# routineLife1/DRBA

Hardware: AMD Instinct MI355X
Metric: interpolated frames/sec @1080p RIFE x2 (higher is better)
Workload: dtype f32 (2xfp16-term MFMA operands = 22 significand bits, fp32 accumulate)

## Files before the change

drba_amd/csrc/conv_split.hip:

```cpp
#include "common.hpp"
#include "conv_split.hpp"

#include <string.h>

#include <map>
#include <mutex>
#include <type_traits>
#include <utility>

using namespace drba;

namespace drba_conv_split {

typedef float f32x4 __attribute__((ext_vector_type(4)));
typedef __bf16 bf16x8 __attribute__((ext_vector_type(8)));
typedef _Float16 f16x8 __attribute__((ext_vector_type(8)));
typedef unsigned u32x4 __attribute__((ext_vector_type(4)));

constexpr int CK = 32;

template <int MODE_, int RW_, int MW_, int NT_, int PL_ = 3, int CS_ = 1, int BP_ = 0>
struct SplitCfg {
  static constexpr int MODE = MODE_, RW = RW_, MW = MW_, NT = NT_, PL = PL_, CS = CS_;
  static constexpr bool BP = BP_ != 0;
  static_assert(!BP || MODE == 1, "row phases exist in the transposed form only");
  static constexpr int NTT = NT * CS;
  static constexpr int NTAP = MODE != 1 ? 9 : 4, NPX = MODE != 1 ? 1 : (BP ? 4 : 2);
  static constexpr int TH = (4 / CS) * RW, TW = 16 * MW, NTC = 16 * NTT;
  static constexpr int TR = MODE == 2 ? 2 * TH + 1 : TH + 2, TC = MODE == 2 ? 2 * TW + 1 : TW + 2, NPIX = TR * TC;
  static constexpr int NPIXP = ((NPIX + 15) / 16) * 16 + 4;
  static constexpr int LDS_BYTES = PL * 4 * NPIXP * 16;
  static constexpr int ITEMS = NPIX * 4;
  static constexpr int LIT = (ITEMS + 255) / 256;
  static constexpr int FRAG_U4 = NTAP * NTT * PL * 64;
#ifndef DRBA_SPLIT_BDEPTH_BIG
#define DRBA_SPLIT_BDEPTH_BIG 2
#endif
#ifndef DRBA_SPLIT_BDEPTH2_BIG
#define DRBA_SPLIT_BDEPTH2_BIG 2
#endif
#ifndef DRBA_SPLIT_BDEPTH2_SMALL
#define DRBA_SPLIT_BDEPTH2_SMALL 4
#endif
  static constexpr int BDEPTH = PL == 3 ? ((RW * MW >= 4) ? DRBA_SPLIT_BDEPTH_BIG : 4)
                                        : ((RW * MW >= 4) ? DRBA_SPLIT_BDEPTH2_BIG : DRBA_SPLIT_BDEPTH2_SMALL);
#ifndef DRBA_SPLIT_MINB3
#define DRBA_SPLIT_MINB3 1
#endif
  static constexpr int MINB = (DRBA_SPLIT_MINB3 && MODE == 0 && RW * MW * NT <= 4 && PL == 3 && CS == 1) ? 3 : 2;
};

__device__ __forceinline__ void split2(float a, float b, unsigned &h, unsigned &m, unsigned &l) {
  typedef __bf16 bf16x2 __attribute__((ext_vector_type(2)));
  typedef float f32x2 __attribute__((ext_vector_type(2)));
  auto pk = [](float x, float y) -> unsigned {
    const bf16x2 p = __builtin_convertvector(f32x2{x, y}, bf16x2);
    return __builtin_bit_cast(unsigned, p);
  };
  h = pk(a, b);
  const float ra = a - __uint_as_float(h << 16), rb = b - __uint_as_float(h & 0xffff0000u);
  m = pk(ra, rb);
  l = pk(ra - __uint_as_float(m << 16), rb - __uint_as_float(m & 0xffff0000u));
}

constexpr int kActShift = drba::kSplitActShift;
__device__ __forceinline__ void split2_f16(float a, float b, unsigned &h, unsigned &l) {
  typedef _Float16 f16x2 __attribute__((ext_vector_type(2)));
  typedef float f32x2 __attribute__((ext_vector_type(2)));
  const f32x2 v = (f32x2){a, b} * (1.f / (float)(1 << kActShift));
  const f16x2 hh = __builtin_convertvector(v, f16x2);
  const f32x2 r = (v - __builtin_convertvector(hh, f32x2)) * 2048.f;
  const f16x2 ll = __builtin_convertvector(r, f16x2);
  h = __builtin_bit_cast(unsigned, hh);
  l = __builtin_bit_cast(unsigned, ll);
}

struct TileCtx {
  int x0, y0, cz, n, py;
};

#ifdef DRBA_PHASE_CLOCKS
__device__ long long g_phase[1024 * 4 * 4];
#define DRBA_CLK(var) const long long var = (long long)__builtin_readcyclecounter()
#define DRBA_CLK_ADD(slot, a, b) clk_acc[slot] += (b) - (a)
#define DRBA_CLK_INIT long long clk_acc[4] = {0, 0, 0, 0}
#define DRBA_CLK_FLUSH                                                                     \
  if (lane == 0 && blockIdx.x < 1024) {                                                    \
    for (int k_ = 0; k_ < 4; ++k_) g_phase[(blockIdx.x * 4 + wave) * 4 + k_] += clk_acc[k_]; \
  }
#else
#define DRBA_CLK(var)
#define DRBA_CLK_ADD(slot, a, b)
#define DRBA_CLK_INIT
#define DRBA_CLK_FLUSH
#endif

__device__ __forceinline__ void lds_barrier() { asm volatile("s_waitcnt lgkmcnt(0)\n\ts_barrier" ::: "memory"); }

template <class Cfg, bool PRE, bool RL = false, bool PSH = false>
__global__ void __launch_bounds__(256, Cfg::MINB)
conv_split_mfma(const float *__restrict__ in, const u32x4 *__restrict__ wfrag, const float *__restrict__ bias,
                const float *__restrict__ beta, const float *__restrict__ res, const float *__restrict__ res2,
                float *__restrict__ out, int Cin, int H, int W, int Cout, int act, float post_slope, float pre_slope,
                int n_ctiles, int nbx, int nby, int total, int pixel_shuffle, int Hi, int Wi, unsigned char *status) {
#if defined(__HIP_DEVICE_COMPILE__)
  constexpr int MODE = Cfg::MODE, NTAP = Cfg::NTAP, NPX = Cfg::NPX;
  constexpr int RW = Cfg::RW, MW = Cfg::MW, NT = Cfg::NT, TH = Cfg::TH, TW = Cfg::TW, TC = Cfg::TC;
  constexpr int NPIX = Cfg::NPIX, NPIXP = Cfg::NPIXP, LIT = Cfg::LIT, PL = Cfg::PL;
  static_assert(PL == 3 || !RL, "the residual is rebuilt exactly only from the three bf16 planes");
  extern __shared__ __attribute__((aligned(16))) u32x4 tile[];

  const int tid = threadIdx.x, lane = tid & 63;
  const int wave = __builtin_amdgcn_readfirstlane(tid >> 6);
  const int m = lane & 15, kq = lane >> 4;
  const size_t HW = (size_t)H * W, HWi = (size_t)Hi * Wi;
  const int nchunks = (Cin + CK - 1) / CK;
  constexpr int CS = Cfg::CS, NTT = Cfg::NTT;
  const int row0 = (CS == 1 ? wave : wave % (4 / CS)) * RW;
  const int nt0 = CS == 1 ? 0 : (wave / (4 / CS)) * NT;

  auto decode = [&](int work) -> TileCtx {
    int t = xcd_band(work, total);
    TileCtx c;
    c.py = 0;
    if (MODE == 1 && !Cfg::BP) {
      c.py = t & 1;
      t >>= 1;
    }
    c.cz = t % n_ctiles;
    t /= n_ctiles;
    const int bx = t % nbx;
    t /= nbx;
    c.x0 = bx * TW, c.y0 = (t % nby) * TH, c.n = t / nby;
    return c;
  };

  const unsigned img_bytes = (unsigned)((size_t)Cin * HWi * 4);
  const __amdgpu_buffer_rsrc_t wrsrc =
      __builtin_amdgcn_make_buffer_rsrc((void *)wfrag, 0, n_ctiles * (MODE != 1 ? 1 : 4) * nchunks * Cfg::FRAG_U4 * 16, 0x00020000);
  float pre[LIT][8];
  auto fetch = [&](const TileCtx &c, int q) {
    const __amdgpu_buffer_rsrc_t irsrc =
        __builtin_amdgcn_make_buffer_rsrc((void *)(in + (size_t)c.n * Cin * HWi), 0, img_bytes, 0x00020000);
    const int plane = (int)HWi * 4;
#pragma unroll
    for (int it = 0; it < LIT; ++it) {
      const int item = tid + 256 * it;
      const int g = item / NPIX, p = item - g * NPIX;
      const int r = p / TC, cc = p - r * TC;
      const int y = (MODE == 2 ? 2 * c.y0 : c.y0) + r - 1, x = (MODE == 2 ? 2 * c.x0 : c.x0) + cc - 1;
      const bool ok = item < Cfg::ITEMS && y >= 0 && y < Hi && x >= 0 && x < Wi;
      const unsigned voff = ok ? (unsigned)(g * 8 * plane + (y * Wi + x) * 4) : 0xffffffffu;
#pragma unroll
      for (int i = 0; i < 8; ++i)
        pre[it][i] = __builtin_bit_cast(float, __builtin_amdgcn_raw_buffer_load_b32(irsrc, voff, (q * CK + i) * plane, 0));
    }
  };
  auto stage = [&]() {
#pragma unroll
    for (int it = 0; it < LIT; ++it) {
      const int item = tid + 256 * it;
      if (item >= Cfg::ITEMS) continue;
      const int g = item / NPIX, slot = g * NPIXP + (item - g * NPIX);
      u32x4 h, mm, l;
#pragma unroll
      for (int i = 0; i < 4; ++i) {
        float a = pre[it][2 * i], b = pre[it][2 * i + 1];
        if (PRE) {
          a = a > 0.f ? a : a * pre_slope;
          b = b > 0.f ? b : b * pre_slope;
        }
        unsigned hh, hm = 0, hl;
        if constexpr (PL == 3) split2(a, b, hh, hm, hl);
        else split2_f16(a, b, hh, hl);
        h[i] = hh, mm[i] = hm, l[i] = hl;
      }
      tile[slot] = h;
      if constexpr (PL == 3) tile[4 * NPIXP + slot] = mm;
      tile[4 * (PL - 1) * NPIXP + slot] = l;
    }
  };

  const bool vec = !PSH && (W & 3) == 0 && (MW & 1) == 0;

  int work = blockIdx.x;
  if (work >= total) return;
  DRBA_CLK_INIT;
  float nf = 0.f;
#ifdef DRBA_SPLIT_STAGGER
  {
    const int b = blockIdx.x;
    const bool late = DRBA_SPLIT_STAGGER == 1 ? (b & 1) : DRBA_SPLIT_STAGGER == 2 ? (b >= (int)gridDim.x / 2) : DRBA_SPLIT_STAGGER == 4 ? ((b >> 8) & 1) : ((b >> 3) & 1);
    if (late) {
      for (int i = 0; i < DRBA_SPLIT_STAGGER_N; ++i) __builtin_amdgcn_s_sleep(127);
    }
  }
#endif
  TileCtx ctx = decode(work);
  auto first_chunk = [&](const TileCtx &c) -> int { return RL ? (c.cz + 1 == nchunks ? 0 : c.cz + 1) : 0; };
  fetch(ctx, first_chunk(ctx));
  while (true) {
    f32x4 acc[NPX][RW][MW][NT];
    f32x4 acl[PL == 2 ? NPX : 1][RW][MW][NT];
#pragma unroll
    for (int p = 0; p < NPX; ++p)
#pragma unroll
      for (int a = 0; a < RW; ++a)
#pragma unroll
        for (int b = 0; b < MW; ++b)
#pragma unroll
          for (int c = 0; c < NT; ++c) {
            acc[p][a][b][c] = (f32x4){0.f, 0.f, 0.f, 0.f};
            if constexpr (PL == 2) acl[p][a][b][c] = (f32x4){0.f, 0.f, 0.f, 0.f};
          }
    const int next = work + (int)gridDim.x;
    TileCtx nctx = ctx;
    if (next < total) nctx = decode(next);
    const bool regroup = MODE != 1 && vec;
    float bs[NT], bt[NT], bs2[NT], bt2[NT];
#pragma unroll
    for (int nt = 0; nt < NT; ++nt) {
      const int co = ctx.cz * Cfg::NTC + (nt0 + nt) * 16 + (regroup ? (lane >> 3) : m), co2 = co + 8;
      bs[nt] = (bias && co < Cout) ? bias[co] : 0.f;
      bt[nt] = (beta && co < Cout) ? beta[co] : 0.f;
      bs2[nt] = (regroup && bias && co2 < Cout) ? bias[co2] : 0.f;
      bt2[nt] = (regroup && beta && co2 < Cout) ? beta[co2] : 0.f;
    }

    for (int qi = 0; qi < nchunks; ++qi) {
      int q = qi;
      if (RL) {
        q = qi + first_chunk(ctx);
        if (q >= nchunks) q -= nchunks;
      }
      constexpr int NTS = NPX * NTAP, STEPS = NTS * NT, D = Cfg::BDEPTH;
      const int wq = ((MODE != 1 ? ctx.cz : ctx.cz * 4 + 2 * ctx.py) * nchunks + q) * (Cfg::FRAG_U4 * 16);
      const int px_bytes = nchunks * (Cfg::FRAG_U4 * 16);
      auto wload = [&](int step, int pl) -> u32x4 {
        const int p = step / (NTAP * NT), r = step - p * (NTAP * NT);
        const int tap = r / NT, nt = r - tap * NT;
        return __builtin_amdgcn_raw_buffer_load_b128(wrsrc, lane * 16, wq + p * px_bytes + ((tap * NTT + nt0 + nt) * PL + pl) * 1024, 0);
      };
      u32x4 bw[D][PL];
#pragma unroll
      for (int d = 0; d < D; ++d)
#pragma unroll
        for (int pl = 0; pl < PL; ++pl) bw[d][pl] = wload(d, pl);
      DRBA_CLK(c_s0);
      lds_barrier();
      stage();
      lds_barrier();
      DRBA_CLK(c_s1);
      DRBA_CLK_ADD(0, c_s0, c_s1);
#ifndef DRBA_EXP_NOFETCH
      if (qi + 1 < nchunks) fetch(ctx, q + 1 == nchunks ? 0 : q + 1);
      else if (next < total) fetch(nctx, first_chunk(nctx));
#endif

      u32x4 af[RW][MW][PL];
      auto load_piece = [&](int ts, int rw, int mw) {
        const int p = ts / NTAP, tap = ts - p * NTAP;
        const int ro = MODE != 1 ? tap / 3 : ((tap >> 1) ? 0 : 1) + (Cfg::BP ? (p >> 1) : ctx.py);
        const int co = MODE != 1 ? tap % 3 : ((tap & 1) ? 0 : 1) + (Cfg::BP ? (p & 1) : p);
        const int slot = MODE == 2 ? kq * NPIXP + (2 * (row0 + rw) + ro) * TC + 2 * (mw * 16 + m) + co
                                   : kq * NPIXP + (row0 + rw + ro) * TC + mw * 16 + m + co;
#pragma unroll
        for (int pl = 0; pl < PL; ++pl) af[rw][mw][pl] = tile[4 * pl * NPIXP + slot];
      };
#pragma unroll
      for (int rw = 0; rw < RW; ++rw)
#pragma unroll
        for (int mw = 0; mw < MW; ++mw) load_piece(0, rw, mw);
#pragma unroll
      for (int ts = 0; ts < NTS; ++ts) {
        const int p = ts / NTAP;
#pragma unroll
        for (int nt = 0; nt < NT; ++nt) {
          const int step = ts * NT + nt;
#pragma unroll
          for (int rw = 0; rw < RW; ++rw)
#pragma unroll
            for (int mw = 0; mw < MW; ++mw) {
              if constexpr (PL == 3) {
                const bf16x8 bh = __builtin_bit_cast(bf16x8, bw[step % D][0]);
                const bf16x8 bm = __builtin_bit_cast(bf16x8, bw[step % D][1]);
                const bf16x8 bl = __builtin_bit_cast(bf16x8, bw[step % D][PL - 1]);
                const bf16x8 ah = __builtin_bit_cast(bf16x8, af[rw][mw][0]);
                const bf16x8 am = __builtin_bit_cast(bf16x8, af[rw][mw][1]);
                const bf16x8 al = __builtin_bit_cast(bf16x8, af[rw][mw][PL - 1]);
                f32x4 c = acc[p][rw][mw][nt];
                c = __builtin_amdgcn_mfma_f32_16x16x32_bf16(al, bh, c, 0, 0, 0);
                c = __builtin_amdgcn_mfma_f32_16x16x32_bf16(ah, bl, c, 0, 0, 0);
                c = __builtin_amdgcn_mfma_f32_16x16x32_bf16(am, bm, c, 0, 0, 0);
                c = __builtin_amdgcn_mfma_f32_16x16x32_bf16(am, bh, c, 0, 0, 0);
                c = __builtin_amdgcn_mfma_f32_16x16x32_bf16(ah, bm, c, 0, 0, 0);
                c = __builtin_amdgcn_mfma_f32_16x16x32_bf16(ah, bh, c, 0, 0, 0);
                acc[p][rw][mw][nt] = c;
              } else {
                const f16x8 bh = __builtin_bit_cast(f16x8, bw[step % D][0]), bl = __builtin_bit_cast(f16x8, bw[step % D][1]);
                const f16x8 ah = __builtin_bit_cast(f16x8, af[rw][mw][0]), al = __builtin_bit_cast(f16x8, af[rw][mw][1]);
                f32x4 c = acl[p][rw][mw][nt];
                c = __builtin_amdgcn_mfma_f32_16x16x32_f16(al, bh, c, 0, 0, 0);
                c = __builtin_amdgcn_mfma_f32_16x16x32_f16(ah, bl, c, 0, 0, 0);
                acl[p][rw][mw][nt] = c;
                acc[p][rw][mw][nt] = __builtin_amdgcn_mfma_f32_16x16x32_f16(ah, bh, acc[p][rw][mw][nt], 0, 0, 0);
              }
#ifndef DRBA_EXP_NOALOAD
              if (nt == NT - 1 && ts + 1 < NTS) load_piece(ts + 1, rw, mw);
#endif
            }
#ifndef DRBA_EXP_NOWLOAD
          if (step + D < STEPS) {
#pragma unroll
            for (int pl = 0; pl < PL; ++pl) bw[step % D][pl] = wload(step + D, pl);
          }
#endif

          __builtin_amdgcn_sched_barrier(0);
        }
      }
      DRBA_CLK(c_m1);
      DRBA_CLK_ADD(1, c_s1, c_m1);
    }
    DRBA_CLK(c_e0);
    if constexpr (PL == 2) {
#pragma unroll
      for (int p = 0; p < NPX; ++p)
#pragma unroll
        for (int a = 0; a < RW; ++a)
#pragma unroll
          for (int b = 0; b < MW; ++b)
#pragma unroll
            for (int c = 0; c < NT; ++c)
            {
              acc[p][a][b][c] = (acc[p][a][b][c] + acl[p][a][b][c] * (1.f / 2048.f)) * (float)(1 << kActShift);
#pragma unroll
              for (int k = 0; k < 4; ++k) nf = nf_fold(nf, acc[p][a][b][c][k]);
            }
    }

    if constexpr (MODE != 1 && PSH) {
      const unsigned obytes = (unsigned)((size_t)Cout * HW * 4);
      const __amdgpu_buffer_rsrc_t orsrc =
          __builtin_amdgcn_make_buffer_rsrc((void *)(out + (size_t)ctx.n * Cout * HW), 0, obytes, 0x00020000);
      auto epilogue_ps = [&](auto post) {
#pragma unroll
        for (int nt = 0; nt < NT; ++nt)
#pragma unroll
          for (int rw = 0; rw < RW; ++rw)
#pragma unroll
            for (int mw = 0; mw < MW; ++mw) {
              f32x4 v = acc[0][rw][mw][nt], o;
              const int co = ctx.cz * Cfg::NTC + (nt0 + nt) * 16 + m;
              const int y = ctx.y0 + row0 + rw;
              const int xb = ctx.x0 + mw * 16 + kq * 4;
              const bool inside = co < Cout && y < H && xb < W;
#pragma unroll
              for (int k = 0; k < 4; ++k) {
                v[k] = post(v[k] + bs[nt]);
                o[k] = quad_xor1(v[k]);
              }
              const int c13 = co >> 2, si = (co >> 1) & 1, sj = co & 1;
              const f32x4 qv = sj ? (f32x4){o[2], v[2], o[3], v[3]} : (f32x4){v[0], o[0], v[1], o[1]};
              const unsigned base = (unsigned)(((c13 * (2 * H) + (2 * y + si)) * (2 * W) + 2 * xb) * 4);
              __builtin_amdgcn_raw_buffer_store_b128(__builtin_bit_cast(u32x4, qv), orsrc, inside ? base + 16u * sj : 0xffffffffu, 0, 0);
            }
      };
      switch (act) {
        case 1: epilogue_ps([](float v) { return lrelu02(v); }); break;
        case 2: epilogue_ps([post_slope](float v) { return v > 0.f ? v : post_slope * v; }); break;
        case 3: epilogue_ps([](float v) { return fmaxf(v, 0.f); }); break;
        case 4: epilogue_ps([](float v) { return tanhf(v) * 10.f; }); break;
        default: epilogue_ps([](float v) { return v; }); break;
      }
    } else if constexpr (MODE != 1) {
      const size_t img = (size_t)ctx.n * Cout * HW;
      if (vec) {
        int ln = lane;
        asm volatile("" : "+v"(ln));
        const int c8 = ln >> 3, blk = (ln >> 2) & 1, q4 = ln & 3;
        const int src = q4 * 16 + blk * 8 + c8;
        const bool hi = (ln & 8) != 0;
        const unsigned obytes = (unsigned)((size_t)Cout * HW * 4);
        const __amdgpu_buffer_rsrc_t orsrc = __builtin_amdgcn_make_buffer_rsrc((void *)(out + img), 0, obytes, 0x00020000);
        const __amdgpu_buffer_rsrc_t rrsrc =
            __builtin_amdgcn_make_buffer_rsrc((void *)((res ? res : out) + img), 0, res ? obytes : 0u, 0x00020000);
        const __amdgpu_buffer_rsrc_t r2rsrc =
            __builtin_amdgcn_make_buffer_rsrc((void *)((res2 ? res2 : out) + img), 0, res2 ? obytes : 0u, 0x00020000);
        auto offs = [&](int nt, int rw, int j, unsigned &oa, unsigned &ob) {
          const int coA = ctx.cz * Cfg::NTC + (nt0 + nt) * 16 + c8;
          const int y = ctx.y0 + row0 + rw;
          const int xb = ctx.x0 + (2 * j + blk) * 16 + q4 * 4;
          const bool in_img = y < H && xb < W;
          const unsigned base = (unsigned)(((coA * H + y) * W + xb) * 4);
          oa = (in_img && coA < Cout) ? base : 0xffffffffu;
          ob = (in_img && coA + 8 < Cout) ? base + 8u * (unsigned)HW * 4u : 0xffffffffu;
        };
        u32x4 ra[2][RW][MW / 2], rb[2][RW][MW / 2];
        auto load_res = [&](int nt) {
#pragma unroll
          for (int rw = 0; rw < RW; ++rw)
#pragma unroll
            for (int j = 0; j < MW / 2; ++j) {
              unsigned oa, ob;
              offs(nt, rw, j, oa, ob);
              ra[nt & 1][rw][j] = __builtin_amdgcn_raw_buffer_load_b128(rrsrc, oa, 0, 0);
              rb[nt & 1][rw][j] = __builtin_amdgcn_raw_buffer_load_b128(rrsrc, ob, 0, 0);
            }
        };
        if (!RL && (res || res2)) load_res(0);
        auto epilogue = [&](auto kind_, auto post) {
          constexpr int KIND = decltype(kind_)::value;
          constexpr bool kBeta = KIND == 3, kRes = !RL && KIND >= 1, kRes2 = !RL && KIND == 2;
#pragma unroll
          for (int nt = 0; nt < NT; ++nt) {
            const float bsA = bs[nt], bsB = bs2[nt], btA = bt[nt], btB = bt2[nt];
            if (kRes && nt + 1 < NT) load_res(nt + 1);
#pragma unroll
            for (int rw = 0; rw < RW; ++rw)
#pragma unroll
              for (int j = 0; j < MW / 2; ++j) {
                const f32x4 v0 = acc[0][rw][2 * j][nt], v1 = acc[0][rw][2 * j + 1][nt];
                f32x4 a, b;
#pragma unroll
                for (int k = 0; k < 4; ++k) {
                  const float got = dpp_f32<0x128>(hi ? v0[k] : v1[k]);
                  a[k] = __shfl(hi ? got : v0[k], src, 64);
                  b[k] = __shfl(hi ? v1[k] : got, src, 64);
                }
                unsigned oa, ob;
                offs(nt, rw, j, oa, ob);
                f32x4 xa = (f32x4){0.f, 0.f, 0.f, 0.f}, xb_ = xa, xa2 = xa, xb2 = xa;
                if (kRes) {
                  xa = __builtin_bit_cast(f32x4, ra[nt & 1][rw][j]);
                  xb_ = __builtin_bit_cast(f32x4, rb[nt & 1][rw][j]);
                }
                if (kRes2) {
                  xa2 = __builtin_bit_cast(f32x4, __builtin_amdgcn_raw_buffer_load_b128(r2rsrc, oa, 0, 0));
                  xb2 = __builtin_bit_cast(f32x4, __builtin_amdgcn_raw_buffer_load_b128(r2rsrc, ob, 0, 0));
                }
                if (RL) {
                  const unsigned short *pl = reinterpret_cast<const unsigned short *>(tile);
                  const int px0 = (row0 + rw + 1) * TC + (2 * j + blk) * 16 + q4 * 4 + 1;
#pragma unroll
                  for (int k = 0; k < 4; ++k) {
                    const int sa = ((2 * nt) * NPIXP + px0 + k) * 8 + c8, sb = sa + NPIXP * 8;
                    const float ha = __uint_as_float((unsigned)pl[sa] << 16), hb = __uint_as_float((unsigned)pl[sb] << 16);
                    const float ma = __uint_as_float((unsigned)pl[4 * NPIXP * 8 + sa] << 16);
                    const float mb = __uint_as_float((unsigned)pl[4 * NPIXP * 8 + sb] << 16);
                    const float la = __uint_as_float((unsigned)pl[8 * NPIXP * 8 + sa] << 16);
                    const float lb = __uint_as_float((unsigned)pl[8 * NPIXP * 8 + sb] << 16);
                    xa[k] = ha + (ma + la);
                    xb_[k] = hb + (mb + lb);
                  }
                }
#pragma unroll
                for (int k = 0; k < 4; ++k) {
                  float ua = a[k] + bsA, ub = b[k] + bsB;
                  if (kBeta) {
                    ua = ua * btA + xa[k];
                    ub = ub * btB + xb_[k];
                  } else {
                    if (RL || kRes) ua = ua + xa[k], ub = ub + xb_[k];
                    if (kRes2) ua = ua + xa2[k], ub = ub + xb2[k];
                  }
                  a[k] = post(ua);
                  b[k] = post(ub);
                }
#ifdef DRBA_EXP_NOSTORE
                if (H >= 0) continue;
#endif
                __builtin_amdgcn_raw_buffer_store_b128(__builtin_bit_cast(u32x4, a), orsrc, oa, 0, 0);
                __builtin_amdgcn_raw_buffer_store_b128(__builtin_bit_cast(u32x4, b), orsrc, ob, 0, 0);
              }
          }
        };
        const float slope = act == 1 ? 0.2f : act == 2 ? post_slope : 1.f;
        auto with_act = [&](auto kind_) {
          if (act == 4) epilogue(kind_, [](float v) { return tanhf(v) * 10.f; });
          else if (act == 3) epilogue(kind_, [](float v) { return v > 0.f ? v : (v != v ? v : 0.f); });
          else epilogue(kind_, [slope](float v) { return v > 0.f ? v : slope * v; });
        };
        if (beta) with_act(std::integral_constant<int, 3>{});
        else if (!RL && res2) with_act(std::integral_constant<int, 2>{});
        else if (RL || res) with_act(std::integral_constant<int, 1>{});
        else with_act(std::integral_constant<int, 0>{});
      } else {
        auto epilogue = [&](auto post) {
#pragma unroll
          for (int nt = 0; nt < NT; ++nt)
#pragma unroll
            for (int rw = 0; rw < RW; ++rw)
#pragma unroll
              for (int mw = 0; mw < MW; ++mw) {
                const f32x4 v = acc[0][rw][mw][nt];
                const int co = ctx.cz * Cfg::NTC + (nt0 + nt) * 16 + m;
                const int y = ctx.y0 + row0 + rw;
                const int xb = ctx.x0 + mw * 16 + kq * 4;
                if (co >= Cout || y >= H || xb >= W) continue;
                const size_t idx = img + ((size_t)co * H + y) * W + xb;
                if ((W & 3) == 0) {
                  f32x4 o, r1 = (f32x4){0.f, 0.f, 0.f, 0.f}, r2 = r1;
                  if (res) r1 = *reinterpret_cast<const f32x4 *>(res + idx);
                  if (res2) r2 = *reinterpret_cast<const f32x4 *>(res2 + idx);
#pragma unroll
                  for (int k = 0; k < 4; ++k) {
                    float u = v[k] + bs[nt];
                    if (beta) u = u * bt[nt] + r1[k];
                    else {
                      if (res) u = u + r1[k];
                      if (res2) u = u + r2[k];
                    }
                    o[k] = post(u);
                  }
                  *reinterpret_cast<f32x4 *>(out + idx) = o;
                  continue;
                }
#pragma unroll
                for (int k = 0; k < 4; ++k) {
                  if (xb + k >= W) continue;
                  float u = v[k] + bs[nt];
                  if (beta) u = u * bt[nt] + res[idx + k];
                  else {
                    if (res) u = u + res[idx + k];
                    if (res2) u = u + res2[idx + k];
                  }
                  out[idx + k] = post(u);
                }
              }
        };
        switch (act) {
          case 1: epilogue([](float v) { return lrelu02(v); }); break;
          case 2: epilogue([post_slope](float v) { return v > 0.f ? v : post_slope * v; }); break;
          case 3: epilogue([](float v) { return fmaxf(v, 0.f); }); break;
          case 4: epilogue([](float v) { return tanhf(v) * 10.f; }); break;
          default: epilogue([](float v) { return v; }); break;
        }
      }
    } else {
      const int Hd = 2 * H, Wd = 2 * W;
      const unsigned obytes = (unsigned)((size_t)Cout * Hd * Wd * 4);
      const __amdgpu_buffer_rsrc_t orsrc =
          __builtin_amdgcn_make_buffer_rsrc((void *)(out + (size_t)ctx.n * Cout * Hd * Wd), 0, obytes, 0x00020000);
      const bool whole = (W & 3) == 0;
      auto epilogue_t = [&](auto ps_) {
        constexpr bool PS = decltype(ps_)::value;
#pragma unroll
        for (int pyi = 0; pyi < (Cfg::BP ? 2 : 1); ++pyi)
#pragma unroll
        for (int rw = 0; rw < RW; ++rw)
#pragma unroll
          for (int mw = 0; mw < MW; ++mw)
#pragma unroll
            for (int nt = 0; nt < NT; ++nt) {
              f32x4 v = acc[Cfg::BP ? 2 * pyi : 0][rw][mw][nt], v1 = acc[Cfg::BP ? 2 * pyi + 1 : NPX - 1][rw][mw][nt];
              const int co = ctx.cz * Cfg::NTC + (nt0 + nt) * 16 + m;
              const int y = ctx.y0 + row0 + rw;
              const int xb = ctx.x0 + mw * 16 + kq * 4;
              const int oy = 2 * y + (Cfg::BP ? pyi : ctx.py);
              const float b0 = bs[nt];
              const bool inside = co < Cout && y < H && xb < W;
#pragma unroll
              for (int k = 0; k < 4; ++k) {
                v[k] += b0;
                v1[k] += b0;
              }
              if constexpr (!PS) {
                const unsigned base = (unsigned)(((co * Hd + oy) * Wd + 2 * xb) * 4);
                if (whole) {
                  const unsigned o = inside ? base : 0xffffffffu;
                  __builtin_amdgcn_raw_buffer_store_b128(__builtin_bit_cast(u32x4, (f32x4){v[0], v1[0], v[1], v1[1]}), orsrc, o, 0, 0);
                  __builtin_amdgcn_raw_buffer_store_b128(__builtin_bit_cast(u32x4, (f32x4){v[2], v1[2], v[3], v1[3]}), orsrc, o, 16, 0);
                } else {
#pragma unroll
                  for (int k = 0; k < 4; ++k) {
                    const unsigned o = (inside && xb + k < W) ? base + 8u * k : 0xffffffffu;
                    __builtin_amdgcn_raw_buffer_store_b32(__float_as_uint(v[k]), orsrc, o, 0, 0);
                    __builtin_amdgcn_raw_buffer_store_b32(__float_as_uint(v1[k]), orsrc, o, 4, 0);
                  }
                }
              } else {
                const int c13 = co >> 2, si = (co >> 1) & 1, sj = co & 1;
                f32x4 o0, o1;
#pragma unroll
                for (int k = 0; k < 4; ++k) {
                  o0[k] = quad_xor1(v[k]);
                  o1[k] = quad_xor1(v1[k]);
                }
                const unsigned base = (unsigned)(((c13 * (2 * Hd) + (2 * oy + si)) * (2 * Wd) + 4 * xb) * 4);
#pragma unroll
                for (int kk = 0; kk < 2; ++kk) {
                  const int k = sj * 2 + kk;
                  const f32x4 qv = sj ? (f32x4){o0[k], v[k], o1[k], v1[k]} : (f32x4){v[k], o0[k], v1[k], o1[k]};
                  const unsigned o = (inside && xb + k < W) ? base + 16u * k : 0xffffffffu;
                  __builtin_amdgcn_raw_buffer_store_b128(__builtin_bit_cast(u32x4, qv), orsrc, o, 0, 0);
                }
              }
            }
      };
      if (pixel_shuffle) epilogue_t(std::true_type{});
      else epilogue_t(std::false_type{});
    }
    DRBA_CLK(c_e1);
    DRBA_CLK_ADD(2, c_e0, c_e1);
    DRBA_CLK_ADD(3, 0, 1);
    if (next >= total) {
      DRBA_CLK_FLUSH;
      break;
    }
    work = next;
    ctx = nctx;
  }
  if constexpr (PL == 2) nf_report(status, DRBA_STATUS_CONV_SPLIT, nf);
#endif
}

using S0 = SplitCfg<0, 1, 2, 2>;
using S1 = SplitCfg<0, 1, 2, 4>;
using S2 = SplitCfg<0, 1, 2, 6>;
using S3 = SplitCfg<0, 1, 4, 2>;
using S4 = SplitCfg<0, 2, 2, 2>;
constexpr int kNum = 5;
using T0 = SplitCfg<1, 1, 2, 2>;
using T1 = SplitCfg<1, 1, 2, 4>;
constexpr int kNumT = 2;
using F0 = SplitCfg<0, 1, 2, 2, 2>;
using F1 = SplitCfg<0, 1, 2, 4, 2>;
using F2 = SplitCfg<0, 1, 2, 6, 2>;
using F3 = SplitCfg<0, 1, 4, 2, 2>;
using F4 = SplitCfg<0, 2, 2, 2, 2>;
using G0 = SplitCfg<1, 1, 2, 2, 2>;
using G1 = SplitCfg<1, 1, 2, 4, 2>;
using X0 = SplitCfg<2, 1, 2, 2, 2>;
using X1 = SplitCfg<2, 1, 2, 4, 2>;
using X2 = SplitCfg<2, 1, 1, 2, 2>;
using X3 = SplitCfg<2, 1, 1, 4, 2>;
constexpr int kNumX = 4;
using Y0 = SplitCfg<0, 2, 2, 2, 2, 2>;
using Y1 = SplitCfg<0, 2, 2, 3, 2, 2>;
using Y2 = SplitCfg<2, 2, 2, 2, 2, 2>;
using Y3 = SplitCfg<2, 2, 1, 2, 2, 2>;
using Y4 = SplitCfg<2, 2, 1, 3, 2, 2>;
using Y5 = SplitCfg<0, 2, 1, 3, 2, 2>;
constexpr int kNumY = 6;
struct Info {
  int NT, NTC, frag_u4, PL;
};
template <class C>
constexpr Info info() {
  return {C::NTT, C::NTC, C::FRAG_U4, C::PL};
}
const Info kInfo[2 * kNum + kNumX + kNumY] = {info<S0>(), info<S1>(), info<S2>(), info<S3>(), info<S4>(),
                                              info<F0>(), info<F1>(), info<F2>(), info<F3>(), info<F4>(),
                                              info<X0>(), info<X1>(), info<X2>(), info<X3>(), info<Y0>(), info<Y1>(), info<Y2>(), info<Y3>(), info<Y4>(), info<Y5>()};
using Z0 = SplitCfg<1, 2, 2, 2, 2, 2>;
using Z1 = SplitCfg<1, 2, 2, 1, 2, 2>;
using Z2 = SplitCfg<1, 2, 2, 1, 2, 2, 1>;
using Z3 = SplitCfg<1, 1, 2, 2, 2, 1, 1>;
using Z4 = SplitCfg<1, 2, 1, 2, 2, 2, 1>;
constexpr int kNumZ = 5;
const Info kInfoT[2 * kNumT + kNumZ] = {info<T0>(), info<T1>(), info<G0>(), info<G1>(), info<Z0>(), info<Z1>(), info<Z2>(), info<Z3>(), info<Z4>()};

template <class Cfg, bool PRE, bool RL = false, bool PSH = false>
hipError_t lds_limit() {
  if (Cfg::LDS_BYTES <= 64 * 1024) return hipSuccess;
  return max_dynamic_lds(reinterpret_cast<const void *>(conv_split_mfma<Cfg, PRE, RL, PSH>), Cfg::LDS_BYTES);
}
template <class Cfg>
constexpr bool kHasShuffle = Cfg::MODE == 0 && Cfg::PL == 2 && Cfg::RW * Cfg::MW == 2 * Cfg::CS && Cfg::NTT == 4 && Cfg::MW == 2;

static int resident_per_cu(const void *kernel, int lds_bytes) {
  static std::mutex mu;
  static std::map<std::pair<const void *, int>, int> known;
  int dev = 0;
  (void)hipGetDevice(&dev);
  std::lock_guard<std::mutex> lock(mu);
  const auto key = std::make_pair(kernel, dev);
  auto it = known.find(key);
  if (it != known.end()) return it->second;
  int occ = 0;
  if (hipOccupancyMaxActiveBlocksPerMultiprocessor(&occ, kernel, 256, lds_bytes) != hipSuccess || occ < 1) occ = 1;
  return known[key] = occ > 3 ? 3 : occ;
}

template <class Cfg>
int launch(const float *in, const float *wpk, const float *bias, const float *beta, const float *res, const float *res2,
           float *out, int N, int Cin, int H, int W, int Cout, int act, float post_slope, int pre_act, float pre_slope,
           int pixel_shuffle, hipStream_t s) {
  const int n_ct = (Cout + Cfg::NTC - 1) / Cfg::NTC;
  const int Hi = H, Wi = W;
  if (Cfg::MODE == 2) H = (Hi - 1) / 2 + 1, W = (Wi - 1) / 2 + 1;
  const int nbx = (W + Cfg::TW - 1) / Cfg::TW, nby = (H + Cfg::TH - 1) / Cfg::TH;
  const long long total = (long long)nbx * nby * N * n_ct * ((Cfg::MODE != 1 || Cfg::BP) ? 1 : 2);
  if (total >= (1ll << 31)) return DRBA_EUNSUPPORTED;
  const u32x4 *wf = reinterpret_cast<const u32x4 *>(wpk);
  unsigned char *status = Cfg::PL == 2 ? status_bytes() : nullptr;
  auto go = [&](auto kernel, hipError_t lds_ok) -> int {
    if (lds_ok != hipSuccess) return DRBA_ELAUNCH;
    const int resident = resident_per_cu(reinterpret_cast<const void *>(kernel), Cfg::LDS_BYTES);
    const int per_cu = env_int("DRBA_SPLIT_PER_CU", resident);
    long long grid = 256ll * per_cu;
    if (grid > total) grid = (total + 7) / 8 * 8;
    DRBA_LAUNCH(kernel, dim3((unsigned)grid), dim3(256), Cfg::LDS_BYTES, s, in, wf, bias, beta, res, res2, out, Cin, H, W, Cout,
                act, post_slope, pre_slope, n_ct, nbx, nby, (int)total, pixel_shuffle, Hi, Wi, status);
    return DRBA_OK;
  };
  int rc;
  if (Cfg::MODE == 0 && pixel_shuffle) {
    if constexpr (kHasShuffle<Cfg>) {
      if (res || res2 || beta || pre_act || (W & 3) || (Cout & 3)) return DRBA_EUNSUPPORTED;
      rc = go(conv_split_mfma<Cfg, false, false, true>, lds_limit<Cfg, false, false, true>());
    } else {
      return DRBA_EUNSUPPORTED;
    }
  } else if constexpr (Cfg::MODE == 0 && Cfg::NTC == CK && Cfg::PL == 3) {
    const bool rl = res && res == in && !res2 && !pre_act && Cin == Cout && (W & 3) == 0;
    rc = rl ? go(conv_split_mfma<Cfg, false, true>, lds_limit<Cfg, false, true>())
            : (pre_act ? go(conv_split_mfma<Cfg, true>, lds_limit<Cfg, true>()) : go(conv_split_mfma<Cfg, false>, lds_limit<Cfg, false>()));
  } else {
    rc = pre_act ? go(conv_split_mfma<Cfg, true>, lds_limit<Cfg, true>()) : go(conv_split_mfma<Cfg, false>, lds_limit<Cfg, false>());
  }
  if (rc != DRBA_OK) return rc;
  DRBA_CHECK_LAUNCH();
  return DRBA_OK;
}

}

namespace drba {

int conv_split_num_cfgs() { return drba_conv_split::kNum; }
int conv_split_f16_first() { return drba_conv_split::kNum; }
int conv_split_s2_first() { return 2 * drba_conv_split::kNum; }
int conv_split_s2_num_cfgs() { return drba_conv_split::kNumX; }
int conv_split_cs_first() { return 2 * drba_conv_split::kNum + drba_conv_split::kNumX; }
int conv_split_cs_num_cfgs() { return drba_conv_split::kNumY; }
int conv_split_cfg_stride(int id) { return (id >= 2 * drba_conv_split::kNum && id != 14 && id != 15 && id < 19) ? 2 : 1; }

bool conv_split_supports(int Cin, int Cout, int id) {
  using namespace drba_conv_split;
  if (id >= 2 * kNum + kNumX)
    return id < 2 * kNum + kNumX + kNumY && Cin > 0 && Cout > 0 && (conv_split_cfg_stride(id) == 2 || Cin % CK == 0);
  if (id >= 2 * kNum) return Cin > 0 && Cout > 0;
  return id >= 0 && Cin > 0 && Cout > 0 && Cin % CK == 0;
}

size_t conv_split_packed_floats(int Cin, int Cout, int id) {
  if (!conv_split_supports(Cin, Cout, id)) return 0;
  const drba_conv_split::Info &c = drba_conv_split::kInfo[id];
  const size_t n_ct = (Cout + c.NTC - 1) / c.NTC, nch = (Cin + drba_conv_split::CK - 1) / drba_conv_split::CK;
  return n_ct * nch * c.frag_u4 * 4;
}

int conv_split_pack(const float *w, float *packed, int Cin, int Cout, int id) {
  using namespace drba_conv_split;
  if (!w || !packed || !conv_split_supports(Cin, Cout, id)) return DRBA_EINVAL;
  const Info &c = kInfo[id];
  if (c.PL == 2 && !two_term_weights_ok(w, (size_t)Cout * Cin * 9)) return DRBA_EUNSUPPORTED;
  const int n_ct = (Cout + c.NTC - 1) / c.NTC, nch = (Cin + CK - 1) / CK;
  memset(packed, 0, sizeof(float) * conv_split_packed_floats(Cin, Cout, id));
  unsigned short *dst = reinterpret_cast<unsigned short *>(packed);
  for (int cz = 0; cz < n_ct; ++cz)
    for (int q = 0; q < nch; ++q)
      for (int tap = 0; tap < 9; ++tap)
        for (int nt = 0; nt < c.NT; ++nt)
          for (int lane = 0; lane < 64; ++lane) {
            const int co = cz * c.NTC + nt * 16 + (lane & 15);
            if (co >= Cout) continue;
            for (int i = 0; i < 8; ++i) {
              const int ci = q * CK + 8 * (lane >> 4) + i;
              if (ci >= Cin) continue;
              unsigned short term[3];
              split_weight_terms(w[((size_t)co * Cin + ci) * 9 + tap], c.PL, term);
              for (int pl = 0; pl < c.PL; ++pl) {
                const size_t unit = ((((size_t)cz * nch + q) * 9 + tap) * c.NT + nt) * c.PL + pl;
                dst[(unit * 64 + lane) * 8 + i] = term[pl];
              }
            }
          }
  return DRBA_OK;
}

int conv_split_launch(int id, const float *in, const float *packed_w, const float *bias, const float *beta,
                      const float *residual, const float *residual2, float *out, int N, int Cin, int H, int W, int Cout,
                      int act, float post_slope, int pre_act, float pre_slope, void *stream, int pixel_shuffle) {
  using namespace drba_conv_split;
  if (!conv_split_supports(Cin, Cout, id)) return DRBA_EUNSUPPORTED;
  if ((size_t)Cin * H * W * 4 >= (1ull << 31)) return DRBA_EUNSUPPORTED;
  if ((size_t)Cout * H * W * 4 >= (1ull << 31)) return DRBA_EUNSUPPORTED;
  hipStream_t s = (hipStream_t)stream;
#define DRBA_CASE(ID, T) \
  case ID:               \
    return launch<T>(in, packed_w, bias, beta, residual, residual2, out, N, Cin, H, W, Cout, act, post_slope, pre_act, \
                     pre_slope, pixel_shuffle, s);
  switch (id) {
    DRBA_CASE(0, S0)
    DRBA_CASE(1, S1)
    DRBA_CASE(2, S2)
    DRBA_CASE(3, S3)
    DRBA_CASE(4, S4)
    DRBA_CASE(5, F0)
    DRBA_CASE(6, F1)
    DRBA_CASE(7, F2)
    DRBA_CASE(8, F3)
    DRBA_CASE(9, F4)
    DRBA_CASE(10, X0)
    DRBA_CASE(11, X1)
    DRBA_CASE(12, X2)
    DRBA_CASE(13, X3)
    DRBA_CASE(14, Y0)
    DRBA_CASE(15, Y1)
    DRBA_CASE(16, Y2)
    DRBA_CASE(17, Y3)
    DRBA_CASE(18, Y4)
    DRBA_CASE(19, Y5)
  }
#undef DRBA_CASE
  return DRBA_EUNSUPPORTED;
}

int deconv_split_num_cfgs() { return drba_conv_split::kNumT; }

int deconv_split_f16_first() { return drba_conv_split::kNumT; }

int deconv_split_total_cfgs() { return 2 * drba_conv_split::kNumT + drba_conv_split::kNumZ; }
bool deconv_split_supports(int Cin, int Cout, int id) {
  return id >= 0 && id < deconv_split_total_cfgs() && Cin > 0 && Cout > 0 && Cin % drba_conv_split::CK == 0;
}

size_t deconv_split_packed_floats(int Cin, int Cout, int id) {
  if (!deconv_split_supports(Cin, Cout, id)) return 0;
  const drba_conv_split::Info &c = drba_conv_split::kInfoT[id];
  const size_t n_ct = (Cout + c.NTC - 1) / c.NTC, nch = Cin / drba_conv_split::CK;
  return n_ct * 4 * nch * c.frag_u4 * 4;
}

int deconv_split_pack(const float *w, float *packed, int Cin, int Cout, int id) {
  using namespace drba_conv_split;
  if (!w || !packed || !deconv_split_supports(Cin, Cout, id)) return DRBA_EINVAL;
  const Info &c = kInfoT[id];
  if (c.PL == 2 && !two_term_weights_ok(w, (size_t)Cin * Cout * 16)) return DRBA_EUNSUPPORTED;
  const int n_ct = (Cout + c.NTC - 1) / c.NTC, nch = Cin / CK;
  memset(packed, 0, sizeof(float) * deconv_split_packed_floats(Cin, Cout, id));
  unsigned short *dst = reinterpret_cast<unsigned short *>(packed);
  for (int cz = 0; cz < n_ct; ++cz)
    for (int phase = 0; phase < 4; ++phase) {
      const int py = phase >> 1, px = phase & 1;
      for (int q = 0; q < nch; ++q)
        for (int tap = 0; tap < 4; ++tap) {
          const int a = tap >> 1, b = tap & 1;
          const int ky = py ? (a ? 2 : 0) : (a ? 3 : 1);
          const int kx = px ? (b ? 2 : 0) : (b ? 3 : 1);
          for (int nt = 0; nt < c.NT; ++nt)
            for (int lane = 0; lane < 64; ++lane) {
              const int co = cz * c.NTC + nt * 16 + (lane & 15);
              if (co >= Cout) continue;
              for (int i = 0; i < 8; ++i) {
                const int ci = q * CK + 8 * (lane >> 4) + i;
                unsigned short term[3];
                split_weight_terms(w[(((size_t)ci * Cout + co) * 4 + ky) * 4 + kx], c.PL, term);
                for (int pl = 0; pl < c.PL; ++pl) {
                  const size_t unit = ((((((size_t)cz * 4 + phase) * nch + q) * 4 + tap) * c.NT + nt) * c.PL + pl);
                  dst[(unit * 64 + lane) * 8 + i] = term[pl];
                }
              }
            }
        }
    }
  return DRBA_OK;
}

int deconv_split_launch(int id, const float *in, const float *packed_w, const float *bias, float *out, int N, int Cin, int H,
                        int W, int Cout, int pixel_shuffle, int pre_act, float pre_slope, void *stream) {
  using namespace drba_conv_split;
  if (!deconv_split_supports(Cin, Cout, id)) return DRBA_EUNSUPPORTED;
  if ((size_t)Cin * H * W * 4 >= (1ull << 31)) return DRBA_EUNSUPPORTED;
  if ((size_t)Cout * 4 * H * W * 4 >= (1ull << 32) - 64) return DRBA_EUNSUPPORTED;
  hipStream_t s = (hipStream_t)stream;
#define DRBA_CASE(ID, T) \
  case ID:               \
    return launch<T>(in, packed_w, bias, nullptr, nullptr, nullptr, out, N, Cin, H, W, Cout, 0, 0.f, pre_act, pre_slope, \
                     pixel_shuffle, s);
  switch (id) {
    DRBA_CASE(0, T0)
    DRBA_CASE(1, T1)
    DRBA_CASE(2, G0)
    DRBA_CASE(3, G1)
    DRBA_CASE(4, Z0)
    DRBA_CASE(5, Z1)
    DRBA_CASE(6, Z2)
    DRBA_CASE(7, Z3)
    DRBA_CASE(8, Z4)
  }
#undef DRBA_CASE
  return DRBA_EUNSUPPORTED;
}

}
```

Baseline: 1194.

## Load input tiles with 128-bit buffer loads and parity-split stride-2 LDS layout

Result: no change. 1194 (-0.1%).

```diff
diff --git a/drba_amd/csrc/conv_split.hip b/drba_amd/csrc/conv_split.hip
--- a/drba_amd/csrc/conv_split.hip
+++ b/drba_amd/csrc/conv_split.hip
@@ -28,10 +28,48 @@
   static constexpr int NTAP = MODE != 1 ? 9 : 4, NPX = MODE != 1 ? 1 : (BP ? 4 : 2);
   static constexpr int TH = (4 / CS) * RW, TW = 16 * MW, NTC = 16 * NTT;
   static constexpr int TR = MODE == 2 ? 2 * TH + 1 : TH + 2, TC = MODE == 2 ? 2 * TW + 1 : TW + 2, NPIX = TR * TC;
-  static constexpr int NPIXP = ((NPIX + 15) / 16) * 16 + 4;
+#ifndef DRBA_SPLIT_PARITY
+#define DRBA_SPLIT_PARITY 1
+#endif
+#ifndef DRBA_SPLIT_WIDE
+#define DRBA_SPLIT_WIDE 1
+#endif
+  static constexpr bool PAR = MODE == 2 && DRBA_SPLIT_PARITY;
+#ifndef DRBA_SPLIT_WGROUP
+#define DRBA_SPLIT_WGROUP 0
+#endif
+  static constexpr bool WG = MODE != 2 && DRBA_SPLIT_WGROUP;
+  static constexpr int EO = TW + 4, TCP = PAR ? EO + TW : (WG ? (TC | 1) : TC);
+  __host__ __device__ static constexpr int cslot(int cc) { return PAR ? ((cc & 1) ? EO + (cc >> 1) : (cc >> 1)) : cc; }
+#ifndef DRBA_SPLIT_KQPAD
+#define DRBA_SPLIT_KQPAD 4
+#endif
+  static constexpr int NPIXP = ((TR * TCP + 15) / 16) * 16 + DRBA_SPLIT_KQPAD;
   static constexpr int LDS_BYTES = PL * 4 * NPIXP * 16;
   static constexpr int ITEMS = NPIX * 4;
   static constexpr int LIT = (ITEMS + 255) / 256;
+  static constexpr bool WIDE_OK = DRBA_SPLIT_WIDE && MW >= 2;
+  static constexpr int NRUN = (TC + 3 + 3) / 4;
+  static constexpr int ITEMS_W = 4 * TR * NRUN;
+  static constexpr int LITW = (ITEMS_W + 255) / 256;
+  __device__ static void wide_item(int item, int &g, int &r, int &j) {
+    constexpr int PER_G = TR * NRUN;
+    g = item / PER_G;
+    const int u = item - g * PER_G;
+    if constexpr (!WG) {
+      r = u / NRUN, j = u - r * NRUN;
+    } else {
+      constexpr int BLK = 4 * NRUN, FULL = (TR / 4) * BLK, PAIRS = (NRUN / 2) * 8;
+      if (u < FULL) {
+        const int b = u / BLK, v = u - b * BLK;
+        if (v < PAIRS) r = 4 * b + ((v >> 1) & 3), j = 2 * (v >> 3) + (v & 1);
+        else r = 4 * b + (v - PAIRS), j = NRUN - 1;
+      } else {
+        const int w = u - FULL, rr = w / NRUN;
+        r = (TR / 4) * 4 + rr, j = w - rr * NRUN;
+      }
+    }
+  }
   static constexpr int FRAG_U4 = NTAP * NTT * PL * 64;
 #ifndef DRBA_SPLIT_BDEPTH_BIG
 #define DRBA_SPLIT_BDEPTH_BIG 2
@@ -97,7 +135,7 @@
 
 __device__ __forceinline__ void lds_barrier() { asm volatile("s_waitcnt lgkmcnt(0)\n\ts_barrier" ::: "memory"); }
 
-template <class Cfg, bool PRE, bool RL = false, bool PSH = false>
+template <class Cfg, bool PRE, bool RL = false, bool PSH = false, bool WIDE = false>
 __global__ void __launch_bounds__(256, Cfg::MINB)
 conv_split_mfma(const float *__restrict__ in, const u32x4 *__restrict__ wfrag, const float *__restrict__ bias,
                 const float *__restrict__ beta, const float *__restrict__ res, const float *__restrict__ res2,
@@ -138,46 +176,84 @@
   const unsigned img_bytes = (unsigned)((size_t)Cin * HWi * 4);
   const __amdgpu_buffer_rsrc_t wrsrc =
       __builtin_amdgcn_make_buffer_rsrc((void *)wfrag, 0, n_ctiles * (MODE != 1 ? 1 : 4) * nchunks * Cfg::FRAG_U4 * 16, 0x00020000);
-  float pre[LIT][8];
+  float pre[WIDE ? Cfg::LITW * 32 : LIT * 8];
   auto fetch = [&](const TileCtx &c, int q) {
     const __amdgpu_buffer_rsrc_t irsrc =
         __builtin_amdgcn_make_buffer_rsrc((void *)(in + (size_t)c.n * Cin * HWi), 0, img_bytes, 0x00020000);
     const int plane = (int)HWi * 4;
-#pragma unroll
-    for (int it = 0; it < LIT; ++it) {
-      const int item = tid + 256 * it;
-      const int g = item / NPIX, p = item - g * NPIX;
-      const int r = p / TC, cc = p - r * TC;
-      const int y = (MODE == 2 ? 2 * c.y0 : c.y0) + r - 1, x = (MODE == 2 ? 2 * c.x0 : c.x0) + cc - 1;
-      const bool ok = item < Cfg::ITEMS && y >= 0 && y < Hi && x >= 0 && x < Wi;
-      const unsigned voff = ok ? (unsigned)(g * 8 * plane + (y * Wi + x) * 4) : 0xffffffffu;
-#pragma unroll
-      for (int i = 0; i < 8; ++i)
-        pre[it][i] = __builtin_bit_cast(float, __builtin_amdgcn_raw_buffer_load_b32(irsrc, voff, (q * CK + i) * plane, 0));
-    }
+    if constexpr (WIDE) {
+#pragma unroll
+      for (int it = 0; it < Cfg::LITW; ++it) {
+        const int item = tid + 256 * it;
+        int g, r, j;
+        Cfg::wide_item(item, g, r, j);
+        const int y = (MODE == 2 ? 2 * c.y0 : c.y0) + r - 1, x = (MODE == 2 ? 2 * c.x0 : c.x0) - 4 + 4 * j;
+        const bool ok = item < Cfg::ITEMS_W && y >= 0 && y < Hi && x >= 0 && x < Wi;
+        const unsigned voff = ok ? (unsigned)(g * 8 * plane + (y * Wi + x) * 4) : 0xffffffffu;
+#pragma unroll
+        for (int i = 0; i < 8; ++i) {
+          const u32x4 v = __builtin_amdgcn_raw_buffer_load_b128(irsrc, voff, (q * CK + i) * plane, 0);
+#pragma unroll
+          for (int k = 0; k < 4; ++k) pre[(it * 8 + i) * 4 + k] = __builtin_bit_cast(float, v[k]);
+        }
+      }
+    } else {
+#pragma unroll
+      for (int it = 0; it < LIT; ++it) {
+        const int item = tid + 256 * it;
+        const int g = item / NPIX, p = item - g * NPIX;
+        const int r = p / TC, cc = p - r * TC;
+        const int y = (MODE == 2 ? 2 * c.y0 : c.y0) + r - 1, x = (MODE == 2 ? 2 * c.x0 : c.x0) + cc - 1;
+        const bool ok = item < Cfg::ITEMS && y >= 0 && y < Hi && x >= 0 && x < Wi;
+        const unsigned voff = ok ? (unsigned)(g * 8 * plane + (y * Wi + x) * 4) : 0xffffffffu;
+#pragma unroll
+        for (int i = 0; i < 8; ++i)
+          pre[it * 8 + i] = __builtin_bit_cast(float, __builtin_amdgcn_raw_buffer_load_b32(irsrc, voff, (q * CK + i) * plane, 0));
+      }
+    }
+  };
+  auto put = [&](int v, int VS, int slot) __attribute__((always_inline)) {
+    u32x4 h, mm, l;
+#pragma unroll
+    for (int i = 0; i < 4; ++i) {
+      float a = pre[v + 2 * i * VS], b = pre[v + (2 * i + 1) * VS];
+      if (PRE) {
+        a = a > 0.f ? a : a * pre_slope;
+        b = b > 0.f ? b : b * pre_slope;
+      }
+      unsigned hh, hm = 0, hl;
+      if constexpr (PL == 3) split2(a, b, hh, hm, hl);
+      else split2_f16(a, b, hh, hl);
+      h[i] = hh, mm[i] = hm, l[i] = hl;
+    }
+    tile[slot] = h;
+    if constexpr (PL == 3) tile[4 * NPIXP + slot] = mm;
+    tile[4 * (PL - 1) * NPIXP + slot] = l;
   };
   auto stage = [&]() {
-#pragma unroll
-    for (int it = 0; it < LIT; ++it) {
-      const int item = tid + 256 * it;
-      if (item >= Cfg::ITEMS) continue;
-      const int g = item / NPIX, slot = g * NPIXP + (item - g * NPIX);
-      u32x4 h, mm, l;
-#pragma unroll
-      for (int i = 0; i < 4; ++i) {
-        float a = pre[it][2 * i], b = pre[it][2 * i + 1];
-        if (PRE) {
-          a = a > 0.f ? a : a * pre_slope;
-          b = b > 0.f ? b : b * pre_slope;
+    if constexpr (WIDE) {
+#pragma unroll
+      for (int it = 0; it < Cfg::LITW; ++it) {
+        const int item = tid + 256 * it;
+        if (item >= Cfg::ITEMS_W) continue;
+        int g, r, j;
+        Cfg::wide_item(item, g, r, j);
+        const int rowslot = g * NPIXP + r * Cfg::TCP;
+#pragma unroll
+        for (int k = 0; k < 4; ++k) {
+          const int cc = 4 * j - 3 + k;
+          if (cc >= 0 && cc < TC) put(it * 32 + k, 4, rowslot + Cfg::cslot(cc));
         }
-        unsigned hh, hm = 0, hl;
-        if constexpr (PL == 3) split2(a, b, hh, hm, hl);
-        else split2_f16(a, b, hh, hl);
-        h[i] = hh, mm[i] = hm, l[i] = hl;
       }
-      tile[slot] = h;
-      if constexpr (PL == 3) tile[4 * NPIXP + slot] = mm;
-      tile[4 * (PL - 1) * NPIXP + slot] = l;
+    } else {
+#pragma unroll
+      for (int it = 0; it < LIT; ++it) {
+        const int item = tid + 256 * it;
+        if (item >= Cfg::ITEMS) continue;
+        const int g = item / NPIX, p = item - g * NPIX;
+        const int r = p / TC, cc = p - r * TC;
+        put(it * 8, 1, g * NPIXP + r * Cfg::TCP + Cfg::cslot(cc));
+      }
     }
   };
 
@@ -262,8 +338,9 @@
         const int p = ts / NTAP, tap = ts - p * NTAP;
         const int ro = MODE != 1 ? tap / 3 : ((tap >> 1) ? 0 : 1) + (Cfg::BP ? (p >> 1) : ctx.py);
         const int co = MODE != 1 ? tap % 3 : ((tap & 1) ? 0 : 1) + (Cfg::BP ? (p & 1) : p);
-        const int slot = MODE == 2 ? kq * NPIXP + (2 * (row0 + rw) + ro) * TC + 2 * (mw * 16 + m) + co
-                                   : kq * NPIXP + (row0 + rw + ro) * TC + mw * 16 + m + co;
+        const int slot = MODE == 2 ? kq * NPIXP + (2 * (row0 + rw) + ro) * Cfg::TCP +
+                                         (Cfg::PAR ? mw * 16 + m + (co == 1 ? Cfg::EO : (co >> 1)) : 2 * (mw * 16 + m) + co)
+                                   : kq * NPIXP + (row0 + rw + ro) * Cfg::TCP + mw * 16 + m + co;
 #pragma unroll
         for (int pl = 0; pl < PL; ++pl) af[rw][mw][pl] = tile[4 * pl * NPIXP + slot];
       };
@@ -441,7 +518,7 @@
                 }
                 if (RL) {
                   const unsigned short *pl = reinterpret_cast<const unsigned short *>(tile);
-                  const int px0 = (row0 + rw + 1) * TC + (2 * j + blk) * 16 + q4 * 4 + 1;
+                  const int px0 = (row0 + rw + 1) * Cfg::TCP + (2 * j + blk) * 16 + q4 * 4 + 1;
 #pragma unroll
                   for (int k = 0; k < 4; ++k) {
                     const int sa = ((2 * nt) * NPIXP + px0 + k) * 8 + c8, sb = sa + NPIXP * 8;
@@ -661,10 +738,10 @@
 constexpr int kNumZ = 5;
 const Info kInfoT[2 * kNumT + kNumZ] = {info<T0>(), info<T1>(), info<G0>(), info<G1>(), info<Z0>(), info<Z1>(), info<Z2>(), info<Z3>(), info<Z4>()};
 
-template <class Cfg, bool PRE, bool RL = false, bool PSH = false>
+template <class Cfg, bool PRE, bool RL = false, bool PSH = false, bool WIDE = false>
 hipError_t lds_limit() {
   if (Cfg::LDS_BYTES <= 64 * 1024) return hipSuccess;
-  return max_dynamic_lds(reinterpret_cast<const void *>(conv_split_mfma<Cfg, PRE, RL, PSH>), Cfg::LDS_BYTES);
+  return max_dynamic_lds(reinterpret_cast<const void *>(conv_split_mfma<Cfg, PRE, RL, PSH, WIDE>), Cfg::LDS_BYTES);
 }
 template <class Cfg>
 constexpr bool kHasShuffle = Cfg::MODE == 0 && Cfg::PL == 2 && Cfg::RW * Cfg::MW == 2 * Cfg::CS && Cfg::NTT == 4 && Cfg::MW == 2;
@@ -705,20 +782,29 @@
                 act, post_slope, pre_slope, n_ct, nbx, nby, (int)total, pixel_shuffle, Hi, Wi, status);
     return DRBA_OK;
   };
+  const bool wide = Cfg::WIDE_OK && (Wi & 3) == 0;
+  auto pick = [&](auto pre_, auto rl_, auto psh_) -> int {
+    constexpr bool P = decltype(pre_)::value, R = decltype(rl_)::value, S = decltype(psh_)::value;
+    if constexpr (Cfg::WIDE_OK) {
+      if (wide) return go(conv_split_mfma<Cfg, P, R, S, true>, lds_limit<Cfg, P, R, S, true>());
+    }
+    return go(conv_split_mfma<Cfg, P, R, S, false>, lds_limit<Cfg, P, R, S, false>());
+  };
+  constexpr std::true_type yes{};
+  constexpr std::false_type no{};
   int rc;
   if (Cfg::MODE == 0 && pixel_shuffle) {
     if constexpr (kHasShuffle<Cfg>) {
       if (res || res2 || beta || pre_act || (W & 3) || (Cout & 3)) return DRBA_EUNSUPPORTED;
-      rc = go(conv_split_mfma<Cfg, false, false, true>, lds_limit<Cfg, false, false, true>());
+      rc = pick(no, no, yes);
     } else {
       return DRBA_EUNSUPPORTED;
     }
   } else if constexpr (Cfg::MODE == 0 && Cfg::NTC == CK && Cfg::PL == 3) {
     const bool rl = res && res == in && !res2 && !pre_act && Cin == Cout && (W & 3) == 0;
-    rc = rl ? go(conv_split_mfma<Cfg, false, true>, lds_limit<Cfg, false, true>())
-            : (pre_act ? go(conv_split_mfma<Cfg, true>, lds_limit<Cfg, true>()) : go(conv_split_mfma<Cfg, false>, lds_limit<Cfg, false>()));
+    rc = rl ? pick(no, yes, no) : (pre_act ? pick(yes, no, no) : pick(no, no, no));
   } else {
-    rc = pre_act ? go(conv_split_mfma<Cfg, true>, lds_limit<Cfg, true>()) : go(conv_split_mfma<Cfg, false>, lds_limit<Cfg, false>());
+    rc = pre_act ? pick(yes, no, no) : pick(no, no, no);
   }
   if (rc != DRBA_OK) return rc;
   DRBA_CHECK_LAUNCH();
@@ -789,10 +875,16 @@
   if ((size_t)Cin * H * W * 4 >= (1ull << 31)) return DRBA_EUNSUPPORTED;
   if ((size_t)Cout * H * W * 4 >= (1ull << 31)) return DRBA_EUNSUPPORTED;
   hipStream_t s = (hipStream_t)stream;
-#define DRBA_CASE(ID, T) \
-  case ID:               \
-    return launch<T>(in, packed_w, bias, beta, residual, residual2, out, N, Cin, H, W, Cout, act, post_slope, pre_act, \
-                     pre_slope, pixel_shuffle, s);
+#ifndef DRBA_SPLIT_BUILD_ID
+#define DRBA_SPLIT_BUILD_ID(id) true
+#define DRBA_SPLIT_BUILD_TID(id) true
+#endif
+#define DRBA_CASE(ID, T)                                                                                                    \
+  case ID:                                                                                                                  \
+    if constexpr (DRBA_SPLIT_BUILD_ID(ID))                                                                                  \
+      return launch<T>(in, packed_w, bias, beta, residual, residual2, out, N, Cin, H, W, Cout, act, post_slope, pre_act,    \
+                       pre_slope, pixel_shuffle, s);                                                                        \
+    break;
   switch (id) {
     DRBA_CASE(0, S0)
     DRBA_CASE(1, S1)
@@ -877,10 +969,12 @@
   if ((size_t)Cin * H * W * 4 >= (1ull << 31)) return DRBA_EUNSUPPORTED;
   if ((size_t)Cout * 4 * H * W * 4 >= (1ull << 32) - 64) return DRBA_EUNSUPPORTED;
   hipStream_t s = (hipStream_t)stream;
-#define DRBA_CASE(ID, T) \
-  case ID:               \
-    return launch<T>(in, packed_w, bias, nullptr, nullptr, nullptr, out, N, Cin, H, W, Cout, 0, 0.f, pre_act, pre_slope, \
-                     pixel_shuffle, s);
+#define DRBA_CASE(ID, T)                                                                                                   \
+  case ID:                                                                                                                 \
+    if constexpr (DRBA_SPLIT_BUILD_TID(ID))                                                                                \
+      return launch<T>(in, packed_w, bias, nullptr, nullptr, nullptr, out, N, Cin, H, W, Cout, 0, 0.f, pre_act, pre_slope, \
+                       pixel_shuffle, s);                                                                                  \
+    break;
   switch (id) {
     DRBA_CASE(0, T0)
     DRBA_CASE(1, T1)
```
